# Freebirdgo/MapReduce_Rust

Hardware: AMD Instinct MI355X
Metric: word-count input GB/s (whole node) at 1/2/4/8 MI355X + % of HBM roofline (higher is better)
Workload: dtype u8

## Files before the change

mapreduce_rust_amd/csrc/k_map.hip:

```cpp
#include "mrg_device.h"
#include "mrg_internal.h"
#include "mrg_split.h"

namespace {

constexpr int NW = MRG_MAP_WAVES;
constexpr int WG = 64 * NW;
constexpr int SEG = MRG_MAP_SEG;
constexpr int TILE = MRG_MAP_TILE;
constexpr int HALO = MRG_MAP_HALO;
constexpr int BEHIND = MRG_MAP_BEHIND;
constexpr int NSUB = MRG_MAP_NSUB;
constexpr int BLK = NSUB * TILE;
constexpr int WIN = BEHIND + TILE + HALO + 48;
constexpr int QCAP = TILE / 2 + 16;
constexpr int NMP = 64;
static_assert(TILE == 64 * SEG, "one segment per lane");
static_assert(WIN % 16 == 0, "16-byte window rows");
static_assert(NMP == TILE / SEG, "one mask pair per segment of the tile");
static_assert(16 * (1 + TILE / 16 + HALO / 16) <= WIN, "staged vectors fit the window row");
static_assert(BEHIND + (TILE - 1) + 31 + 20 <= WIN, "the 5-dword key read stays in the window row");
static_assert(BEHIND == 16 && HALO % 16 == 0 && HALO >= 64, "one 16-byte vector behind, whole halo vectors");
static_assert(QCAP >= TILE / 2 + 1, "the token queue holds every start of a tile");
static_assert(BLK == 2 * TILE && NSUB == 2, "A/B register sets hold two tiles per lane (v0, v1)");
// ... 33 lines not shown
    __builtin_amdgcn_wave_barrier();
    __builtin_amdgcn_fence(__ATOMIC_ACQUIRE, "wavefront");
}

#define GAS __attribute__((address_space(1)))
template <class T>
__device__ __forceinline__ GAS T *gp(T *p) {
    return (GAS T *)p;
}
#define CAS __attribute__((address_space(4)))
template <class T>
__device__ __forceinline__ const CAS T *cp(const T *p) {
    return (const CAS T *)p;
}
typedef uint32_t u32x4 __attribute__((ext_vector_type(4)));
typedef uint64_t u64x2 __attribute__((ext_vector_type(2)));
typedef uint32_t u32x3a __attribute__((ext_vector_type(3), aligned(4)));
typedef uint32_t u32x4u __attribute__((ext_vector_type(4), aligned(1)));
typedef uint32_t u32u __attribute__((aligned(1)));
template <class T>
__device__ __forceinline__ T g_add(T *p, T v) {
    return __hip_atomic_fetch_add(gp(p), v, __ATOMIC_RELAXED, __HIP_MEMORY_SCOPE_AGENT);
}
__device__ __forceinline__ uint64_t umin64(uint64_t a, uint64_t b) { return a < b ? a : b; }
__device__ __forceinline__ uint64_t umax64(uint64_t a, uint64_t b) { return a > b ? a : b; }

struct TileInfo {
    uint64_t At, t0, t1, doc_lo, doc_hi, wlo, whi;
    uint32_t docid, v0, v1;
};

struct BlkInfo {
    uint64_t Ab, doc_lo, doc_hi;
    uint32_t docid, v0, v1;
};

__device__ __forceinline__ BlkInfo locate_blk(const MapArgs &A, uint64_t c, uint32_t &d) {
    const CAS uint64_t *cb = cp(A.chunk_base), *doff = cp(A.doc_off);
    while (cb[d + 1] <= c) ++d;
    BlkInfo b;
    b.doc_lo = doff[d];
    b.doc_hi = doff[d + 1];
    b.Ab = (b.doc_lo & ~15ull) + (c - cb[d]) * (uint64_t)BLK;
    b.docid = A.doc_id ? cp(A.doc_id)[d] : d;
    const uint64_t vbase = b.Ab - (uint64_t)BEHIND;
    const uint64_t wlo = umax64(b.doc_lo, b.Ab >= (uint64_t)BEHIND ? b.Ab - BEHIND : 0ull);
    const uint64_t whi = umin64(b.Ab + (uint64_t)(BLK + HALO), b.doc_hi);
    b.v0 = (uint32_t)(((wlo & ~15ull) - vbase) >> 4);
    b.v1 = (uint32_t)((((whi + 15u) & ~15ull) - vbase) >> 4);
    return b;
}

__device__ __forceinline__ uint32_t find_doc(const MapArgs &A, uint64_t c) {
    const CAS uint64_t *cb = cp(A.chunk_base);
    uint32_t lo = 0, hi = A.n_docs;
    while (hi - lo > 1) {
        const uint32_t mid = (lo + hi) >> 1;
        if (cb[mid] <= c) lo = mid;
        else hi = mid;
    }
    return lo;
}

__device__ __forceinline__ TileInfo sub_tile(const BlkInfo &b, uint32_t j) {
    TileInfo t;
    t.At = b.Ab + (uint64_t)j * TILE;
    t.doc_lo = b.doc_lo;
    t.doc_hi = b.doc_hi;
    t.docid = b.docid;
    t.t0 = umax64(t.At, t.doc_lo);
    t.t1 = umin64(t.At + (uint64_t)TILE, t.doc_hi);
    const uint64_t wbase = t.At - (uint64_t)BEHIND;
    t.wlo = umax64(t.doc_lo, t.At >= (uint64_t)BEHIND ? t.At - BEHIND : 0ull);
    t.whi = umin64(t.t1 + (uint64_t)HALO, t.doc_hi);
    t.v0 = (uint32_t)(((t.wlo & ~15ull) - wbase) >> 4);
// ... 442 lines not shown
        for (int t = 0; t < N; ++t) idx[t] = atomicAdd(&(w16[t] ? R.cur16 : R.cur)[b[t]], tl[t] ? 1ull : 0ull);
    } else {
#pragma unroll
        for (int t = 0; t < N; ++t) idx[t] = 0;
    }
    bool anyo = false, ovf[N];
#pragma unroll
    for (int t = 0; t < N; ++t) {
        const bool ok = tl[t] && idx[t] < end[t];
        if (ok) store_tail<IDX>(pool, pool16, w16[t], idx[t], k0[t], k1[t], docid);
        ovf[t] = tl[t] && !ok;
        anyo = anyo || ovf[t];
    }
    if (__any(anyo)) {
#pragma unroll
        for (int t = 0; t < N; ++t)
            if (ovf[t]) ovf_append<IDX>(A, b[t], k0[t], k1[t], docid);
    }
    }
}

template <int CAP, bool IDX, bool WIDE, bool T64>
__device__ __forceinline__ void emit(const MapArgs &A, LdsTable<CAP, IDX> &table, TailRegions R, bool have,
                                     uint64_t tk0, uint64_t tk1, uint32_t tlen, uint64_t tstart, uint32_t traw,
                                     uint32_t docid) {
    const bool is_long = have && tlen > 16u;
    if constexpr (WIDE) {
        wide_store(A, R, have && !is_long, tk0, tk1);
    } else {
    bool tail = false;
    uint32_t h = 0;
    const uint32_t dkey = IDX ? docid : MRG_EMPTY_DOC;
    if (have && !is_long) {
        h = key_hash(tk0, tk1, dkey, A.hash_bits);
    }
    {
        const bool act = have && !is_long && !(map_ablate(A) & 2u);
        tail = (have && !is_long) && !table.insert_wave(act, tk0, tk1, dkey, h);
    }
    if (tail && !(map_ablate(A) & 1u)) {
        const uint32_t b = bucket_of(h);
        const bool w16 = !IDX && (T64 ? (uint32_t)tk1 != 0u : key_over12(tk1));
        if constexpr (!T64) {
            if (w16) {
                tail16_append(A, R, gp(A.pool16), b, tk0, tk1);
            } else {
                const uint64_t ce = atomicAdd(&R.cur[b], 1ull);
                const uint32_t i = (uint32_t)ce;
                if (i < (uint32_t)(ce >> 32)) store_tail32<IDX>(gp(A.pool), i, tk0, tk1, docid);
                else ovf_append<IDX>(A, b, tk0, tk1, docid);
            }
        } else {
        const uint64_t end = (w16 ? R.end16 : R.end)[b];
        const uint64_t idx = atomicAdd(&(w16 ? R.cur16 : R.cur)[b], 1ull);
        if (idx < end) store_tail<IDX>(gp(A.pool), gp(A.pool16), w16, idx, tk0, tk1, docid);
        else ovf_append<IDX>(A, b, tk0, tk1, docid);
        }
    }
    }
    if (__any(is_long)) {
        const uint64_t mask = __ballot(is_long);
        const int leader = __ffsll((long long)mask) - 1;
        uint32_t base = 0;
        if ((int)__lane_id() == leader) base = atomicAdd(R.lcnt, (unsigned int)__popcll(mask));
        base = (uint32_t)__builtin_amdgcn_readlane((int)base, leader);
        const uint32_t k = base + (uint32_t)__popcll(mask & mrg_lanemask_lt());
        if (is_long) {
// ... 83 lines not shown
#define LDS __attribute__((address_space(3)))
__device__ __forceinline__ uint32_t uni_class(const LDS uint8_t *uc, uint32_t cp) {
    uint32_t byte;
    if (cp < 0x800u) byte = uc[cp >> 2];
    else if ((cp >> 8) == 0x20u) byte = uc[512u + ((cp & 255u) >> 2)];
    else return mrg_uclass(cp);
    return (byte >> (2u * (cp & 3u))) & 3u;
}
template <int CAP, bool IDX, bool WIDE, bool T64>
__global__ __launch_bounds__(WG, 1) void k_map(const MapArgs *__restrict__ Ap) {
    const MapArgs &A = *Ap;
    constexpr bool BQ = !IDX && !WIDE;
    constexpr int WROW = BQ ? WINB : WIN, QROW = BQ ? QCAPB : QCAP;
    __shared__ __attribute__((aligned(16))) uint8_t s_win[NW][WROW];
    __shared__ __attribute__((aligned(8))) uint32_t s_mp[NW][BQ ? NMWB : 2 * NMP];
    __shared__ __attribute__((aligned(8))) uint16_t s_q[NW][QROW];
    static_assert((QROW * sizeof(uint16_t)) % 8 == 0 && QROW * sizeof(uint16_t) >= 64 * 8, "queue rows hold 64 u64 slots");
    __shared__ __attribute__((aligned(1024))) uint8_t s_lut[4][256];
    __shared__ __attribute__((aligned(16))) uint32_t s_sel[17 * 17][4];
    __shared__ KeyPair s_key[WIDE ? 2 : CAP];
    __shared__ unsigned int s_cnt[WIDE ? 2 : CAP];
    __shared__ __attribute__((aligned(16))) unsigned int s_doc[IDX ? CAP : 1];
    __shared__ unsigned long long s_tcur[WIDE ? 1 : MRG_NBUCKET];
    __shared__ unsigned long long s_tend[(WIDE || !T64) ? 1 : MRG_NBUCKET];
    __shared__ unsigned long long s_tcur16[(IDX || WIDE) ? 1 : MRG_NBUCKET];
    __shared__ unsigned long long s_tend16[(IDX || WIDE || !T64) ? 1 : MRG_NBUCKET];
    __shared__ uint32_t s_hist[WIDE ? 1 : MRG_NBUCKET + 1];
    __shared__ unsigned int s_wcur[WIDE ? MRG_WMAP_MAXB1 : 1];
    __shared__ __attribute__((aligned(16))) uint64_t s_wspl[WIDE ? 2 * MRG_WMAP_MAXB1 : 1];
    __shared__ __attribute__((aligned(4))) uint8_t s_wix[WIDE ? MRG_WMAP_IXR * MRG_WIDE_IX1 : 4];
    __shared__ uint32_t s_next, s_ngen;
    __shared__ uint32_t s_stolen;
    __shared__ uint32_t s_share[2];
    __shared__ uint32_t s_pool[NW];
    __shared__ uint32_t s_nuni;
    __shared__ uint8_t s_uc[9 * 64];
    __shared__ uint32_t s_tot[3];
    __shared__ unsigned int s_fill;
    __shared__ unsigned int s_lcnt;
    __shared__ unsigned int s_door[(MRG_MAP_DOOR && !WIDE) ? LdsTable<CAP, IDX>::DW : 1];
    static_assert(WIDE || sizeof(s_q) >= CAP * sizeof(uint16_t), "flush ranks reuse the queues");
    static_assert((CAP & (CAP - 1)) == 0 && CAP >= 64 && CAP <= 65536, "2-way sets: NS = CAP / 2 a power of two, ranks in u16");
    static_assert(sizeof(s_door) / sizeof(s_door[0]) >= ((MRG_MAP_DOOR && !WIDE) ? LdsTable<CAP, IDX>::DW : 1u), "doorkeeper words");
    static_assert(!WIDE || (sizeof(s_wcur) / sizeof(s_wcur[0]) == MRG_WMAP_MAXB1 && sizeof(s_wspl) / sizeof(s_wspl[0]) == 2 * MRG_WMAP_MAXB1 &&
                            sizeof(s_wix) == MRG_WMAP_IXR * MRG_WIDE_IX1 && MRG_WIDE_IX1 % 4 == 0),
                  "wide map: cursors, splitters and index rows as the host plan sizes them");
    if constexpr (WIDE) {
        if (A.wR * A.wB1r > (uint32_t)MRG_WMAP_MAXB1 || A.wB1r == 0u || (A.wix && A.wR > (uint32_t)MRG_WMAP_IXR)) return;
    }

    const int tid = threadIdx.x;
    const int lane = tid & 63, wv = __builtin_amdgcn_readfirstlane(tid >> 6);
    if constexpr (WIDE) {
        const uint32_t nb1 = A.wR * A.wB1r, nsp = 2u * A.wR * (A.wB1r - 1u);
        for (uint32_t b = tid; b < nb1; b += WG) s_wcur[b] = 0;
        for (uint32_t i = tid; i < nsp; i += WG) s_wspl[i] = gp(A.wspl)[i];
        if (A.wix)
            for (uint32_t i = tid; i < A.wR * (MRG_WIDE_IX1 / 4); i += WG)
                reinterpret_cast<uint32_t *>(s_wix)[i] = gp(reinterpret_cast<const uint32_t *>(A.wix))[i];
    }
    for (int i = tid; i < (WIDE ? 2 : CAP); i += WG) {
        s_key[i] = KeyPair{MRG_EMPTY_K0, MRG_EMPTY_K1};
        s_cnt[i] = 0;
        if (IDX) s_doc[i] = MRG_EMPTY_DOC;
    }
    if (MRG_MAP_DOOR && !WIDE)
// ... 29 lines not shown
        s_tot[1] = 0;
        s_tot[2] = 0;
        s_fill = 0;
        s_lcnt = 0;
    }
    for (int i = tid; i < 9 * 64; i += WG) {
        const uint32_t blk = i < 512 ? (uint32_t)i >> 6 : 0x20u;
        s_uc[i] = c_uclass_stage2[c_uclass_stage1[blk] * 64u + ((uint32_t)i & 63u)];
    }
    for (int i = tid; i < 1024; i += WG) {
        const uint32_t v = (uint32_t)i & 255u, c = mrg_uclass(v & 127u);
        const uint32_t ws = v >= 128u ? 0x11u : ((c == MRG_CLS_W ? 1u : 0u) | (c == MRG_CLS_S ? 0x10u : 0u));
        s_lut[i >> 8][v] = (uint8_t)(ws << (i >> 8));
    }
    auto zmask = [](uint32_t L, uint32_t j) {
        uint32_t m = 0;
        for (uint32_t p = 0; p < 4; ++p)
            if (4u * j + 3u - p >= L) m |= 0xFFu << (8u * p);
        return m;
    };
    for (int i = tid; i < 17 * 17 * 4; i += WG) {
        const uint32_t L = (uint32_t)i / 68u, g = ((uint32_t)i / 4u) % 17u, j = (uint32_t)i & 3u;
        const uint32_t zm = zmask(L, j), gm = zmask(g, j);
        s_sel[L * 17u + g][j] = ((0x00010203u + (gm & 0x01010101u)) & ~zm) | (0x0C0C0C0Cu & zm);
    }
    LdsTable<CAP, IDX> table{s_key, s_cnt, s_doc, s_door, &s_fill};
    const TailRegions tails{s_tcur, s_tend, s_tcur16, s_tend16, &s_lcnt, s_wcur, s_wspl, A.wix ? s_wix : nullptr};
    uint32_t my_tokens = 0;
#ifdef MRG_MAP_ABLATION
    const uint32_t abl = A.ablate;
#else
    constexpr uint32_t abl = MRG_MAP_ABL_CONST;
#endif
    const uint32_t hbits = A.hash_bits;
    GAS uint64_t *const pool = gp(A.pool);
    GAS uint64_t *const pool16 = gp(A.pool16);
    uint8_t *win = s_win[wv];
    uint32_t *mw = s_mp[wv];
    uint64_t *mp = reinterpret_cast<uint64_t *>(s_mp[wv]);
    uint16_t *queue = s_q[wv];
    __syncthreads();

    const uint32_t j0 = 1u + (uint32_t)lane;
    const uint32_t j1 = lane == 0 ? 0u : 64u + (uint32_t)lane;
    const bool has1 = lane < 5;
    auto load = [&](const TileInfo &t, uint4 &p0, uint4 &p1) {
        const GAS u32x4 *src = reinterpret_cast<const GAS u32x4 *>(gp(A.in) + (t.At - (uint64_t)BEHIND));
        u32x4 v0 = {0, 0, 0, 0}, v1 = {0, 0, 0, 0};
        if (j0 >= t.v0 && j0 < t.v1) v0 = src[j0];
        if (has1 && j1 >= t.v0 && j1 < t.v1) v1 = src[j1];
        p0 = uint4{v0.x, v0.y, v0.z, v0.w};
        p1 = uint4{v1.x, v1.y, v1.z, v1.w};
    };
    struct Blk {
        uint4 v0, v1, e;
    };
#ifdef MRG_MAP_ABLATION
    BlkInfo first_blk{};
#endif
    auto load_blk = [&](const BlkInfo &b0, Blk &X) {
#ifdef MRG_MAP_ABLATION
        const BlkInfo &b = (abl & 8u) ? first_blk : b0;
#else
        const BlkInfo &b = b0;
#endif
        const GAS uint8_t *src = gp(A.in) + (b.Ab - (uint64_t)BEHIND);
        auto ld = [&](uint32_t idx) -> uint4 {
            const u32x4 t = __builtin_nontemporal_load(reinterpret_cast<const GAS u32x4 *>(src + 16u * min(max(idx, b.v0), b.v1 - 1u)));
            return uint4{t.x, t.y, t.z, t.w};
        };
        X.v0 = ld(1u + (uint32_t)lane);
        X.v1 = ld(65u + (uint32_t)lane);
        X.e = ld(lane == 0 ? 0u : 128u + (uint32_t)lane);
    };

    GAS uint32_t *glist = gp(A.gbits) + (uint64_t)blockIdx.x * A.kwords;

#ifdef MRG_MAP_PROF
    const bool P = A.prof != nullptr;
    uint64_t pacc[7] = {0, 0, 0, 0, 0, 0, 0}, tl = P ? clock64() : 0;
    const uint64_t wg_t0 = wall_clock64();
    unsigned long long ftv[5] = {0, 0, 0, 0, 0};
#define MRG_FT(i)                                   \
    if (P && tid == 0) ftv[i] = wall_clock64();
#define MRG_PT(i)                          \
    if (P) {                               \
        const uint64_t t_ = clock64();     \
        pacc[i] += t_ - tl;                \
        tl = t_;                           \
    }
#else
#define MRG_PT(i)
#define MRG_FT(i)
#endif
    auto extract = [&](uint32_t q, uint32_t sraw, uint32_t total, bool &fast, bool &slow, uint32_t &s,
                       uint64_t &tk0, uint64_t &tk1) -> uint32_t {
        const bool act = q < total;
        s = act ? sraw : 0u;
        uint32_t Wp, Sp;
        if constexpr (BQ) {
            const uint32_t ma = mw[s >> 4], mb = mw[(s >> 4) + 1u];
            Wp = __builtin_amdgcn_perm(mb, ma, 0x05040100u);
            Sp = __builtin_amdgcn_perm(mb, ma, 0x07060302u);
        } else {
            const uint64_t pr = mp[s >> 4];
            Wp = (uint32_t)pr;
            Sp = (uint32_t)(pr >> 32);
        }
        const uint32_t i = s & 15u;
// ... 71 lines not shown
                const uint32_t r = (uint32_t)__builtin_ctz(~(W >> b));
                W &= ~(((1u << r) - 1u) << b);
                const uint32_t off = (uint32_t)BEHIND + 16u * seg + b;
                const uint32_t dw = off >> 2, ra = off & 3u;
                const uint32_t d0 = win32[dw], d1 = win32[dw + 1], d2 = win32[dw + 2], d3 = win32[dw + 3],
                               d4 = win32[dw + 4];
                const u32x4 sl = *reinterpret_cast<const u32x4 *>(s_sel[r * 17u + 16u]);
                const uint32_t a0 = __builtin_amdgcn_alignbyte(d1, d0, ra), a1 = __builtin_amdgcn_alignbyte(d2, d1, ra),
                               a2 = __builtin_amdgcn_alignbyte(d3, d2, ra), a3 = __builtin_amdgcn_alignbyte(d4, d3, ra),
                               a4 = __builtin_amdgcn_alignbyte(0u, d4, ra);
                const uint64_t v0 = ((uint64_t)__builtin_amdgcn_perm(a1, a0, sl.x) << 32) | __builtin_amdgcn_perm(a2, a1, sl.y);
                const uint64_t v1 = ((uint64_t)__builtin_amdgcn_perm(a3, a2, sl.z) << 32) | __builtin_amdgcn_perm(a4, a3, sl.w);
                const uint32_t ks = 8u * tlen;
                if (ks == 0u) {
                    tk0 |= v0;
                    tk1 |= v1;
                } else if (ks < 64u) {
                    tk0 |= v0 >> ks;
                    tk1 |= (v1 >> ks) | (v0 << (64u - ks));
                } else {
                    tk1 |= v0 >> (ks - 64u);
                }
                tlen += r;
            }
            tlen += (uint32_t)__builtin_popcount(W);
            if (S) {
                traw = 16u * seg + e - s;
                return true;
            }
        }
        return false;
    };

    auto process_blk = [&](const BlkInfo &I, const Blk &X, uint32_t cblk, auto &&mid) {
        const uint64_t Ab = I.Ab, doc_lo = I.doc_lo, doc_hi = I.doc_hi;
        const uint32_t docid = I.docid;
        const uint32_t lo_rel = doc_lo > Ab ? (uint32_t)(doc_lo - Ab) : 0u;
        const uint32_t hi_rel = (uint32_t)umin64(doc_hi - Ab, (uint64_t)(BLK + HALO));
        const bool edge = lo_rel != 0u || hi_rel != (uint32_t)(BLK + HALO);
        auto clip = [&](uint32_t m, uint32_t B) -> uint32_t {
            const uint32_t lo_inv = lo_rel > B ? min(lo_rel - B, 16u) : 0u;
            const uint32_t hi_ok = B < hi_rel ? min(hi_rel - B, 16u) : 0u;
            const uint32_t valid = ((1u << hi_ok) - 1u) & ~((1u << lo_inv) - 1u);
            return (m & (valid | (valid << 16))) | ((~valid & 0xFFFFu) << 16);
        };
        auto classify = [&](const uint4 &x) -> uint32_t {
            uint32_t e[16];
#pragma unroll
            for (int k = 0; k < 4; ++k) {
                const uint32_t w = k == 0 ? x.x : (k == 1 ? x.y : (k == 2 ? x.z : x.w));
#pragma unroll
                for (int b = 0; b < 4; ++b)
                    e[4 * k + b] = s_lut[b][b == 0 ? (w & 0xFFu) : (b == 3 ? w >> 24 : __builtin_amdgcn_ubfe(w, 8 * b, 8))];
            }
            uint32_t yk[4];
#pragma unroll
            for (int k = 0; k < 4; ++k) yk[k] = e[4 * k] | e[4 * k + 1] | e[4 * k + 2] | e[4 * k + 3];
            const uint32_t y = (yk[0] | (yk[1] << 8)) | ((yk[2] | (yk[3] << 8)) << 16);
            const uint32_t t = y & 0x0F0F0F0Fu, u = (y >> 4) & 0x0F0F0F0Fu;
            return __builtin_amdgcn_perm(u | (u >> 4), t | (t >> 4), 0x06040200u);
        };
        auto na = [](const uint4 &x) { return ((x.x | x.y | x.z | x.w) & 0x80808080u) != 0u; };
        const uint32_t l16 = (uint32_t)lane * SEG;
        uint32_t m0 = classify(X.v0), m1 = classify(X.v1);
        uint32_t mh;
        {
            const uint32_t e0 = lane_u32(X.e.x, 1), e1 = lane_u32(X.e.y, 1), e2 = lane_u32(X.e.z, 1),
                           e3 = lane_u32(X.e.w, 1);
            const uint32_t k = (uint32_t)lane & 15u;
            const uint32_t dwv = k < 8u ? (k < 4u ? e0 : e1) : (k < 12u ? e2 : e3);
            const uint32_t cl = s_lut[0][__builtin_amdgcn_ubfe(dwv, 8u * (k & 3u), 8)];
            const uint32_t wm = (uint32_t)__ballot(lane < 16 && (cl & 1u));
            const uint32_t sm = (uint32_t)__ballot(lane < 16 && (cl & 0x10u));
            mh = (wm & 0xFFFFu) | (sm << 16);
        }
        if (edge) {
            m0 = clip(m0, l16);
            m1 = clip(m1, 1024u + l16);
            mh = clip(mh, (uint32_t)BLK);
        }
        const bool n0 = na(X.v0), n1 = na(X.v1), ne = na(X.e);
        uint32_t prev_blk =
            Ab > doc_lo ? (uint32_t)(s_lut[0][lane_u32(X.e.w, 0) >> 24] >> 4) & 1u : 1u;
        bool defer_blk = false;
        if (!(abl & 256u) && !(MRG_MAP_ABL_CONST & 0x20000u) && __any(n0 || n1 || (lane <= 1 && ne))) {
#ifdef MRG_MAP_NO_UNI
            defer_blk = true;
#else
            const int64_t dlo = (int64_t)(doc_lo - Ab);
            const int lo = (int)(dlo < -(int64_t)BEHIND ? -(int64_t)BEHIND : dlo);
            const int hi = (int)umin64(doc_hi - Ab, (uint64_t)(BLK + HALO));
            const LDS uint8_t *uc = (const LDS uint8_t *)s_uc;
            bool bad = false;
            auto hb = [](uint32_t d) { return ((((d & 0x80808080u) >> 7) * 0x00204081u) >> 21) & 0xFu; };
            auto nam_of = [](uint32_t m) { return m & (m >> 16) & 0xFFFFu; };
            auto leads = [&](const uint4 &x, uint32_t nam) {
                return (hb(x.x & (x.x << 1)) | (hb(x.y & (x.y << 1)) << 4) | (hb(x.z & (x.z << 1)) << 8) |
                        (hb(x.w & (x.w << 1)) << 12)) & nam;
            };
            const uint32_t nam0 = nam_of(m0), nam1 = nam_of(m1), namh_w = nam_of(mh);
            const uint32_t ld0 = leads(X.v0, nam0), ld1 = leads(X.v1, nam1);
            uint4 xh{0u, 0u, 0u, 0u};
            uint32_t namh = 0u, ldh = 0u;
            if (namh_w) {
                xh = uint4{lane_u32(X.e.x, 1), lane_u32(X.e.y, 1), lane_u32(X.e.z, 1), lane_u32(X.e.w, 1)};
                if (lane == 63) {
                    namh = namh_w;
                    ldh = leads(xh, namh);
                }
            }
            const uint32_t before = lane_u32(X.e.w, 0);
            int pbp = 0;
            bool has_b = false;
            if (dlo < 0 && (before >> 24) >= 0x80u) {
                uint32_t bb = before >> 24;
                pbp = -1;
                for (int k = 2; k <= 4 && (bb & 0xC0u) == 0x80u; ++k) {
                    bb = (before >> (8 * (4 - k))) & 0xFFu;
                    pbp = -k;
                }
                if (bb < 0xC0u || pbp < lo) bad = true;
                else has_b = true;
            }
            const uint32_t v1_first = lane_u32(X.v1.x, 0), halo_next = lane_u32(X.e.x, 2);
            uint32_t nA = from_next_lane(X.v0.x), nB = from_next_lane(X.v1.x);
            if (lane == 63) {
                nA = v1_first;
                nB = xh.x;
            }
            auto dec = [&](uint32_t p, uint32_t d0, uint32_t d1, uint32_t d2, uint32_t d3, uint32_t d4, int so,
                           uint32_t &W, uint32_t &S, uint32_t &C) {
                const uint32_t k = p >> 2;
                const uint32_t a = (k & 2u) ? ((k & 1u) ? d3 : d2) : ((k & 1u) ? d1 : d0);
                const uint32_t b = (k & 2u) ? ((k & 1u) ? d4 : d3) : ((k & 1u) ? d2 : d1);
                const uint32_t w = __builtin_amdgcn_alignbyte(b, a, p & 3u);
                auto rd = [&](uint64_t x) -> uint32_t { return (w >> (8u * (uint32_t)x)) & 0xFFu; };
                uint32_t cp = 0, raw;
                const int n = mrg_utf8_decode(rd, 0ull, (uint64_t)min(hi - (so + (int)p), 4), &cp, &raw);
                bad |= n == 0;
                const uint32_t span = ((1u << n) - 1u) << p;
                const uint32_t cl = uni_class(uc, cp);
                C |= span;
                W |= cl == MRG_CLS_W ? span : 0u;
                S |= cl == MRG_CLS_S ? span : 0u;
            };
            uint32_t W0 = 0, S0 = 0, C0 = 0, W1 = 0, S1 = 0, C1 = 0;
            uint32_t mAB0 = (MRG_MAP_ABL_CONST & 0x10000u) ? 0u : (ld0 | (ld1 << 16));
// ... 94 lines not shown
                Wh = WE;
                Sh = SE;
                Ch = CE;
            }
            const uint32_t sp0 = pack(W0, S0, C0), sp1 = pack(W1, S1, C1);
            uint32_t in0 = from_prev_lane(sp0), in1 = from_prev_lane(sp1);
            const uint32_t sp0_last = lane_u32(sp0, 63);
            if (lane == 0) {
                in0 = bsp;
                in1 = sp0_last;
            }
            auto fix = [&](uint32_t m, uint32_t nam, uint32_t W, uint32_t S, uint32_t C, uint32_t in) -> uint32_t {
                W = (W | ((in >> 4) & 0xFu)) & 0xFFFFu;
                S = (S | ((in >> 8) & 0xFu)) & 0xFFFFu;
                C = (C | (in & 0xFu)) & 0xFFFFu;
                if (!(MRG_MAP_ABL_CONST & 0x10000u)) bad |= C != nam;
                return ((m & 0xFFFFu & ~nam) | W) | ((((m >> 16) & ~nam) | S) << 16);
            };
            m0 = fix(m0, nam0, W0, S0, C0, in0);
            m1 = fix(m1, nam1, W1, S1, C1, in1);
            uint32_t mh_l = mh;
            if (lane == 63) mh_l = fix(mh, namh, Wh, Sh, Ch, sp1);
            mh = lane_u32(mh_l, 63);
            prev_blk = lane_u32(pb_l, 0);
            defer_blk = __any(bad);
            if (!defer_blk && lane == 0) atomicAdd(&s_nuni, Ab + (uint64_t)TILE < doc_hi ? 2u : 1u);
#endif
        }
        MRG_PT(1);
        mid();
        MRG_PT(0);
        if (defer_blk) {
            if (lane == 0) {
                for (uint32_t j = 0; j < NSUB && Ab + (uint64_t)j * TILE < doc_hi; ++j) {
                    const uint32_t k = atomicAdd(&s_ngen, 1u);
                    if (k < A.kwords) glist[k] = (uint32_t)(cblk * NSUB + j);
                }
            }
            return;
        }
        if (abl & 32u) {
            my_tokens += (m0 ^ m1 ^ mh ^ prev_blk) & 1u;
            return;
        }

        auto rounds = [&](uint32_t total, bool may_claim) -> uint32_t {
            uint32_t nslow = 0;
            for (uint32_t base = 0; base < total; base += 128) {
                bool fa, sa, fb, sb;
                uint32_t sA, sB;
                uint64_t a0, a1, b0, b1;
                const uint32_t qa = base + (uint32_t)lane, qb = qa + 64u;
                const uint32_t ra = queue[min(qa, (uint32_t)QROW - 1u)], rb = queue[min(qb, (uint32_t)QROW - 1u)];
                uint32_t ga = extract(qa, ra, total, fa, sa, sA, a0, a1);
                uint32_t gb = extract(qb, rb, total, fb, sb, sB, b0, b1);
                if (!(abl & 1024u) && __any((ga | gb) != 0u)) {
                    squeeze(ga, a0, a1);
                    squeeze(gb, b0, b1);
                }
                const uint64_t ma = __ballot(sa), mb = __ballot(sb);
                if (ma | mb) {
                    const uint32_t ra = __builtin_amdgcn_mbcnt_hi((uint32_t)(ma >> 32), __builtin_amdgcn_mbcnt_lo((uint32_t)ma, 0u));
                    const uint32_t rb = __builtin_amdgcn_mbcnt_hi((uint32_t)(mb >> 32), __builtin_amdgcn_mbcnt_lo((uint32_t)mb, 0u));
                    const uint32_t na = (uint32_t)__builtin_popcountll(ma);
                    if (sa) queue[nslow + ra] = (uint16_t)sA;
                    if (sb) queue[nslow + na + rb] = (uint16_t)sB;
// ... 17 lines not shown
            wave_sync_lds();
            auto rd = [&](uint64_t a) -> uint32_t {
                if (a >= At && a < whi) return (uint32_t)win[a - wbase];
                return (uint32_t)gp(A.in)[a];
            };
            for (uint32_t base = 0; base < nslow; base += 64) {
                const uint32_t q = base + (uint32_t)lane;
                bool have = false;
                uint64_t tk0 = 0, tk1 = 0, a = 0;
                uint32_t tlen = 0, traw = 0;
                if (q < nslow) {
                    const uint32_t s = queue[q];
                    a = At + s;
                    if (!(abl & 128u) && mask_walk(s, nseg, tk0, tk1, tlen, traw)) {
                        have = tlen > 0;
                    } else {
                        uint64_t e2;
                        if (walk_token(rd, a, doc_hi, A.counters, tk0, tk1, tlen, e2) && tlen > 0) {
                            have = true;
                            traw = (uint32_t)(e2 - a);
                        }
                    }
                }
                my_tokens += have ? 1u : 0u;
                emit<CAP, IDX, WIDE, T64>(A, table, tails, have, tk0, tk1, tlen, a, traw, docid);
            }
        };
        auto table_open = [&]() -> bool {
            return __builtin_amdgcn_readfirstlane(__hip_atomic_load(&s_fill, __ATOMIC_RELAXED, __HIP_MEMORY_SCOPE_WORKGROUP)) <
                   (uint32_t)CAP;
        };

        if constexpr (BQ) {
            const uint64_t whi = umin64(Ab + (uint64_t)(BLK + HALO), doc_hi);
            wave_sync_lds();
            reinterpret_cast<uint4 *>(win)[1 + lane] = X.v0;
            reinterpret_cast<uint4 *>(win)[65 + lane] = X.v1;
            if (lane >= 1 && lane < 5) reinterpret_cast<uint4 *>(win)[128 + lane] = X.e;
            mw[lane] = m0;
            mw[64 + lane] = m1;
            if (lane == 0) mw[2 * 64] = mh;
            uint32_t pv0 = from_prev_lane(m0) >> 31, pv1 = from_prev_lane(m1) >> 31;
            const uint32_t m0_last = lane_u32(m0, 63) >> 31;
            if (lane == 0) {
                pv0 = prev_blk;
                pv1 = m0_last;
            }
            const uint32_t S0 = m0 >> 16, S1 = m1 >> 16;
            uint32_t st0 = ~S0 & ((S0 << 1) | pv0) & 0xFFFFu;
            uint32_t st1 = ~S1 & ((S1 << 1) | pv1) & 0xFFFFu;
            if (abl & 64u) {
                my_tokens += (st0 ^ st1) & 1u;
                st0 = 0;
                st1 = 0;
            }
            my_tokens += (abl & 4u) ? (uint32_t)__builtin_popcount(st0 | (st1 << 16)) : 0u;
            uint32_t pos0, pos1;
            auto scan2 = [&](uint32_t a0, uint32_t a1) -> uint32_t {
                const uint32_t c0 = (uint32_t)__builtin_popcount(a0), c1 = (uint32_t)__builtin_popcount(a1);
                const uint32_t incl = wave_incl_scan(c0 | (c1 << 16));
                const uint32_t tot = lane_u32(incl, 63);
                pos0 = (incl & 0xFFFFu) - c0;
                pos1 = (tot & 0xFFFFu) + (incl >> 16) - c1;
                return (abl & 68u) ? 0u : (tot & 0xFFFFu) + (tot >> 16);
            };
            auto in_range = [&](uint32_t lo, uint32_t hi, uint32_t &a0, uint32_t &a1) {
                const uint32_t g0 = (uint32_t)lane, g1 = 64u + (uint32_t)lane;
                a0 = g0 >= lo && g0 < hi ? st0 : 0u;
                a1 = g1 >= lo && g1 < hi ? st1 : 0u;
            };
            uint32_t a0 = st0, a1 = st1, seg_hi = BLK / SEG;
            uint32_t total = scan2(a0, a1);
            if (total > (uint32_t)QCAPB) {
                seg_hi = QRANGE;
                in_range(0u, seg_hi, a0, a1);
                total = scan2(a0, a1);
            }
// ... 84 lines not shown
        const uint64_t c0 = (uint64_t)first_u32(s_share[0]) + (uint64_t)first_u32(r);
        if (c0 < (uint64_t)whi_b) {
            run_cur = (uint32_t)c0 + 1u;
            run_end = (uint32_t)umin64(c0 + R, (uint64_t)whi_b);
            return (uint32_t)c0;
        }
        const uint64_t ns2 = A.n_static, np = A.n_chunks - ns2;
        wave_sync_lds();
        uint32_t pt = first_u32(s_pool[wv]);
        while ((pt >> 8) < 8u) {
            const uint32_t part = pt & 7u;
            uint32_t k = 0;
            if (lane == 0) k = atomicAdd(&s_stolen, (uint32_t)MRG_MAP_STEAL_K);
            if (first_u32(k) + (uint32_t)MRG_MAP_STEAL_K > A.steal_max) {
                pt = 8u << 8;
                break;
            }
            const uint32_t plo = (uint32_t)(np * part / 8u), phi = (uint32_t)(np * (part + 1u) / 8u);
            unsigned long long q = 0;
            if (lane == 0) q = atomicAdd(&A.pool_ctr[16u * part], (unsigned long long)MRG_MAP_STEAL_K);
            const uint32_t at = plo + first_u32((uint32_t)umin64(q, 0xFFFFFFFFull));
            if (at < phi) {
                if (lane == 0) s_pool[wv] = pt;
                run_cur = (uint32_t)ns2 + at + 1u;
                run_end = (uint32_t)ns2 + min(phi, at + (uint32_t)MRG_MAP_STEAL_K);
                if (cp(A.chunk_base)[dcur] > ns2 + at) dcur = find_doc(A, ns2 + at);
                return (uint32_t)ns2 + at;
            }
            pt = ((pt & 7u) + 1u) % 8u | (((pt >> 8) + 1u) << 8);
        }
        if (lane == 0) s_pool[wv] = pt;
        return NONE;
    };
    auto next_blk = [&](const BlkInfo &P, uint32_t cp_, uint32_t cn) -> BlkInfo {
        if (cn != cp_ + 1u || P.Ab + (uint64_t)BLK >= P.doc_hi) return locate_blk(A, cn, dcur);
        BlkInfo b = P;
        b.Ab = P.Ab + (uint64_t)BLK;
        const uint64_t whi = umin64(b.Ab + (uint64_t)(BLK + HALO), b.doc_hi);
        b.v0 = 0u;
        b.v1 = (uint32_t)((((whi + 15u) & ~15ull) - (b.Ab - (uint64_t)BEHIND)) >> 4);
        return b;
    };
    uint32_t c = grab();
    if (c != NONE) dcur = find_doc(A, c);
    Blk XA, XB;
    BlkInfo IA{}, IB{};
    auto settle = [](Blk &X) {
        asm volatile("" : "+v"(X.v0.x), "+v"(X.v0.y), "+v"(X.v0.z), "+v"(X.v0.w), "+v"(X.v1.x), "+v"(X.v1.y),
                     "+v"(X.v1.z), "+v"(X.v1.w), "+v"(X.e.x), "+v"(X.e.y), "+v"(X.e.z), "+v"(X.e.w));
    };
    if (c != NONE) {
        IA = locate_blk(A, c, dcur);
#ifdef MRG_MAP_ABLATION
        first_blk = IA;
#endif
        load_blk(IA, XA);
        settle(XA);
    }
    while (c != NONE) {
        const uint32_t cB = grab();
        IB = cB != NONE ? next_blk(IA, c, cB) : IA;
        load_blk(IB, XB);
        process_blk(IA, XA, c, [&]() { settle(XB); });
        c = cB;
        if (c == NONE) break;
        const uint32_t cA = grab();
        IA = cA != NONE ? next_blk(IB, c, cA) : IB;
        load_blk(IA, XA);
        process_blk(IB, XB, c, [&]() { settle(XA); });
        c = cA;
    }
    MRG_PT(4);
#ifdef MRG_MAP_PROF
    __shared__ unsigned long long s_loop_end;
    if (tid == 0) s_loop_end = 0;
    lds_only_barrier();
    if (P && lane == 0) atomicMax(&s_loop_end, (unsigned long long)wall_clock64());
#endif
    lds_only_barrier();
    if (s_ngen) __syncthreads();
    {
        const uint32_t ng = min(s_ngen, A.kwords);
        for (uint32_t i = (uint32_t)wv; i < ng; i += NW) {
            {
                const uint32_t kk = first_u32(glist[i]);
                const uint64_t cb = kk / NSUB;
                uint32_t dgen = find_doc(A, cb);
                const BlkInfo b = locate_blk(A, cb, dgen);
                const TileInfo T = sub_tile(b, kk % NSUB);
                uint4 x0, x1;
                load(T, x0, x1);
                wave_sync_lds();
                if (j0 >= T.v0 && j0 < T.v1) reinterpret_cast<uint4 *>(win)[j0] = x0;
                if (has1 && j1 >= T.v0 && j1 < T.v1) reinterpret_cast<uint4 *>(win)[j1] = x1;
                wave_sync_lds();
                my_tokens += generic_tile<CAP, IDX, WIDE, T64>(A, table, tails, win, T.At, T.t0, T.t1,
                                                    T.doc_lo, T.doc_hi, T.wlo, T.whi, T.docid);
            }
        }
    }

    MRG_PT(5);
    lds_only_barrier();
    uint32_t my_tail = 0, my_tail16 = 0;
    if constexpr (WIDE) {
        uint32_t over = 0;
        for (uint32_t b = tid; b < A.wR * A.wB1r; b += WG) {
            const uint32_t n = s_wcur[b];
            gp(A.wcnt)[(uint64_t)b * gridDim.x + blockIdx.x] = n;
            my_tail += n;
            over += n > A.wcap ? n - A.wcap : 0u;
        }
        if (over) g_add(&A.counters[CNT_OVF], (unsigned long long)over);
    } else {
    uint16_t *s_rank = &s_q[0][0];
    GAS uint32_t *bcount = gp(A.bcount) + (uint64_t)blockIdx.x * MRG_NBUCKET;
    for (int b = tid; b < MRG_NBUCKET; b += WG) {
        const uint32_t n = T64 ? (uint32_t)(s_tcur[b] - (s_tend[b] - gp(A.bcap)[b]))
                               : (uint32_t)s_tcur[b] - ((uint32_t)(s_tcur[b] >> 32) - gp(A.bcap)[b]);
        my_tail += n;
        bcount[b] = n;
        if (!IDX) {
            const uint32_t n16 = T64 ? (uint32_t)(s_tcur16[b] - (s_tend16[b] - gp(A.bcap16)[b]))
                                     : (uint32_t)s_tcur16[b] - ((uint32_t)(s_tcur16[b] >> 32) - gp(A.bcap16)[b]);
            my_tail += n16;
            my_tail16 += n16;
            gp(A.bcount16)[(uint64_t)blockIdx.x * MRG_NBUCKET + b] = n16;
        }
    }
    for (int b = tid; b <= MRG_NBUCKET; b += WG) s_hist[b] = 0;
    lds_only_barrier();
    MRG_FT(0);
    for (int i = tid; i < CAP; i += WG) {
        const KeyPair k = s_key[i];
        if (k.a == MRG_EMPTY_K0) continue;
        const uint32_t b = bucket_of(key_hash(k.a, k.b, IDX ? s_doc[i] : MRG_EMPTY_DOC, A.hash_bits));
        s_rank[i] = (uint16_t)atomicAdd(&s_hist[b], 1u);
    }
    lds_only_barrier();
    MRG_FT(1);
    if (tid < 64) {
        uint32_t run = 0;
        for (int b0 = 0; b0 < MRG_NBUCKET; b0 += 64) {
            const uint32_t v = s_hist[b0 + lane];
            const uint32_t inc = wave_incl_scan(v);
            s_hist[b0 + lane] = run + inc - v;
            run += lane_u32(inc, 63);
        }
        if (lane == 0) s_hist[MRG_NBUCKET] = run;
    }
    lds_only_barrier();
    MRG_FT(2);
    GAS uint32_t *foff = gp(A.foff) + (uint64_t)blockIdx.x * (MRG_NBUCKET + 1);
    for (int b = tid; b <= MRG_NBUCKET; b += WG) foff[b] = s_hist[b];
    const uint64_t reg = (uint64_t)blockIdx.x * CAP;
    for (int i = tid; i < CAP; i += WG) {
        const KeyPair k = s_key[i];
        if (k.a == MRG_EMPTY_K0) continue;
        const uint32_t d = IDX ? s_doc[i] : MRG_EMPTY_DOC;
        const uint32_t b = bucket_of(key_hash(k.a, k.b, d, A.hash_bits));
        const uint64_t pos2 = reg + s_hist[b] + s_rank[i];
        gp(A.fk0)[pos2] = k.a;
        gp(A.fk1)[pos2] = k.b;
        gp(A.fcnt)[pos2] = s_cnt[i];
        if (IDX) gp(A.fdoc)[pos2] = d;
    }
    }
    MRG_FT(3);
    uint32_t t = my_tokens, ttl = my_tail, t16 = my_tail16;
    for (int off = 32; off > 0; off >>= 1) {
        t += __shfl_down(t, off);
        ttl += __shfl_down(ttl, off);
        t16 += __shfl_down(t16, off);
    }
    if (lane == 0) {
        atomicAdd(&s_tot[0], t);
        atomicAdd(&s_tot[1], ttl);
        if (t16) atomicAdd(&s_tot[2], t16);
    }
    lds_only_barrier();
    if (tid == 0) {
        g_add(&A.counters[CNT_TOKENS], (unsigned long long)s_tot[0]);
        g_add(&A.counters[CNT_REC], (unsigned long long)s_tot[1]);
        if (s_tot[2]) g_add(&A.counters[CNT_REC16], (unsigned long long)s_tot[2]);
        if (s_ngen + s_nuni) g_add(&A.counters[CNT_NONASCII], (unsigned long long)(s_ngen + s_nuni));
        if (s_ngen > A.kwords) g_add(&A.counters[CNT_OVF], (unsigned long long)(s_ngen - A.kwords));
        gp(A.lcount)[blockIdx.x] = s_lcnt;
        if (s_lcnt) g_add(&A.counters[CNT_LONG], (unsigned long long)s_lcnt);
    }
    MRG_FT(4);
    MRG_PT(6);
#ifdef MRG_MAP_PROF
    if (P && lane == 0) {
// ... 165 lines not shown
```

mapreduce_rust_amd/csrc/mrgpu.cpp:

```cpp
#include <sys/stat.h>

#include <rccl/rccl.h>

#include <fcntl.h>
#include <unistd.h>

#include <atomic>
#include <condition_variable>
#include <exception>
#include <memory>
#include <thread>

#include "mrg_host.h"

using namespace mrg_host;

static_assert(sizeof(XRec) == MRG_XREC_BYTES, "exchange record layout (include/mrgpu.h)");

thread_local std::string mrg_host::g_err;

DeviceCache &DeviceCache::get() {
    static DeviceCache *c = new DeviceCache();
    return *c;
}
// ... 1121 lines not shown
        uint64_t *d_rbase16 = att.get<uint64_t>(MRG_NBUCKET);
        uint32_t *d_bcap16 = att.get<uint32_t>(MRG_NBUCKET);
        A.bcount16 = att.get<uint32_t>((uint64_t)grid * MRG_NBUCKET);
        MapArgs *dargs = att.get<MapArgs>(1);
        if (ocap > 0xFFFFFFF0ull) raise(MRG_ENOMEM, "input too large for one map launch");
        A.ovf = att.get<uint64_t>((uint64_t)MRG_NBUCKET * ocap * RW);
        A.onext = att.get<uint32_t>(MRG_NBUCKET);
        A.ocap = (uint32_t)ocap;
        stage_fill(c, A.onext, 0, 4ull * MRG_NBUCKET);
        stage_h2d(c, d_rbase, rbase.data(), 8ull * MRG_NBUCKET);
        stage_h2d(c, d_bcap, bcap32.data(), 4ull * MRG_NBUCKET);
        stage_h2d(c, d_rbase16, rbase16.data(), 8ull * MRG_NBUCKET);
        stage_h2d(c, d_bcap16, bcap16_32.data(), 4ull * MRG_NBUCKET);
        A.rbase = d_rbase; A.bcap = d_bcap; A.rbase16 = d_rbase16; A.bcap16 = d_bcap16;
        A.pool = att.get<uint64_t>((rtot * MRG_TAIL_BYTES(idx) + 16 + 7) / 8);
        A.pool16 = att.get<uint64_t>(2 * rtot16 + 2);
        A.fk0 = att.get<uint64_t>((uint64_t)grid * cap);
        A.fk1 = att.get<uint64_t>((uint64_t)grid * cap);
        A.fcnt = att.get<uint32_t>((uint64_t)grid * cap);
        A.fdoc = idx ? att.get<uint32_t>((uint64_t)grid * cap) : nullptr;
        A.foff = att.get<uint32_t>((uint64_t)grid * (MRG_NBUCKET + 1));
        const uint64_t lslots = map_args_shared(c, att, A, in, ms, lcap, launches == 0, launches);
        A.ablate = getenv("MRG_ABLATE") ? (uint32_t)atoi(getenv("MRG_ABLATE")) : 0u;
        A.prof = nullptr;
        if (getenv("MRG_PROF")) {
            A.prof = att.get<unsigned long long>(8 + 8ull * grid);
            HIPCHK(hipMemsetAsync(A.prof, 0, 8ull * (8 + 8ull * grid), s));
        }
        stage_fill(c, c->d_cnt, 0, sizeof(unsigned long long) * CNT_N);
        stage_fill(c, &c->d_cnt[CNT_ERRPOS], 0xFF, sizeof(unsigned long long));
        stage_h2d(c, dargs, &A, sizeof(MapArgs));
        flush_stage(c);
        ev_rec(c, c->ev, 0);
        const bool tail64 = !map_tail_packed(rtot, rtot16, ms) || env_u64("MRG_TEST_TAIL64", 0) != 0;
        mrg_launch_map(nullptr, dargs, c->app, grid, c->lds_cap, s, false, tail64);
        ev_rec(c, c->ev, 1);
        HIPCHK(hipGetLastError());
        ++launches;
        if (launches == 1 && !idx && (c->spec_agg || cold_repeats) && !A.prof && !wide_forced() &&
            !getenv("MRG_NO_SPEC_AGG") && grid <= 2048) {
            ev_rec(c, c->ev, 2);
            uint32_t nsub = c->agg_nsub;
            if (const uint64_t t = env_u64("MRG_TEST_AGG_NSUB", 0)) nsub = (uint32_t)t;
            const bool c32 = c->spec_agg ? c->spec_c32 : true;
            spec = agg_launch(c, A, (uint32_t)grid, cap, agg_ocap(c), nsub, lslots, c32 && grid <= 512, false);
        }
        uint32_t *onext = (uint32_t *)&c->h_cnt[CNT_N + 8];
        HIPCHK(hipMemcpyAsync(onext, A.onext, 4ull * MRG_NBUCKET, hipMemcpyDeviceToHost, s));
        read_counters(c);
        c->st.map_spill = 0;
        for (int b = 0; b < MRG_NBUCKET; ++b) c->st.map_spill += std::min<uint64_t>(onext[b], ocap);
        if (A.prof) {
            unsigned long long pr[8];
            HIPCHK(hipMemcpy(pr, A.prof, sizeof pr, hipMemcpyDeviceToHost));
            double tot = 0;
            for (int i = 0; i < 7; ++i) tot += (double)pr[i];
            static const char *nm[7] = {"load-wait", "classify", "stage+scan+queue", "token rounds", "slow tokens",
                                        "non-ascii", "flush"};
            fprintf(stderr, "[mrgpu] map phase clocks (sum over waves %.3e):", tot);
            for (int i = 0; i < 7; ++i) fprintf(stderr, " %s %.1f%%", nm[i], 100.0 * (double)pr[i] / (tot > 0 ? tot : 1));
            fprintf(stderr, "\n");
            std::vector<unsigned long long> wt(8ull * grid);
            HIPCHK(hipMemcpy(wt.data(), A.prof + 8, 8ull * wt.size(), hipMemcpyDeviceToHost));
            if (wt[1]) {
                unsigned long long t0 = ~0ull, t1 = 0, ls = 0;
                std::vector<double> dur(grid), end(grid), lend(grid);
                std::vector<std::vector<double>> fst(5, std::vector<double>(grid, 0.0));
// ... 2058 lines not shown
```

Before: 1468.

## Slim per-block state in map loop and specialize hash bits on tail mode

Replaces the two full BlkInfo register sets in the double-buffered map loop with one compact CurBlk. When the next chunk is not the consecutive one, its metadata is passed through a small per-wave LDS slot and read back as scalars. It also makes hash_bits a compile-time zero for the packed-tail variant (the host forces the 64-bit tail path whenever hash_bits is nonzero), and uses opaque lane values to simplify lane predicates. The aim is lower VGPR/SGPR pressure and fewer 64-bit ops in the hot loop, at the cost of an extra LDS round-trip and wave sync on non-consecutive chunk switches.

```diff
diff --git a/mapreduce_rust_amd/csrc/k_map.hip b/mapreduce_rust_amd/csrc/k_map.hip
--- a/mapreduce_rust_amd/csrc/k_map.hip
+++ b/mapreduce_rust_amd/csrc/k_map.hip
@@ -89,8 +89,23 @@
 
 struct BlkInfo {
     uint64_t Ab, doc_lo, doc_hi;
-    uint32_t docid, v0, v1;
+    uint32_t docid, v0, v1, cend;
 };
+
+struct CurBlk {
+    uint64_t Ab, doc_hi;
+    int32_t lo;
+    uint32_t docid;
+    uint32_t cend;
+};
+__device__ __forceinline__ CurBlk cur_of(const BlkInfo &b) {
+    const int64_t d = (int64_t)(b.doc_lo - b.Ab);
+    return CurBlk{b.Ab, b.doc_hi, (int32_t)(d < -(int64_t)BEHIND ? -(int64_t)BEHIND : d), b.docid, b.cend};
+}
+__device__ __forceinline__ uint32_t clip_u32(uint64_t x, uint32_t m) {
+    const uint32_t l = (uint32_t)(x >> 32) ? 0xFFFFFFFFu : (uint32_t)x;
+    return l < m ? l : m;
+}
 
 __device__ __forceinline__ BlkInfo locate_blk(const MapArgs &A, uint64_t c, uint32_t &d) {
     const CAS uint64_t *cb = cp(A.chunk_base), *doff = cp(A.doc_off);
@@ -98,6 +113,7 @@
     BlkInfo b;
     b.doc_lo = doff[d];
     b.doc_hi = doff[d + 1];
+    b.cend = (uint32_t)cb[d + 1];
     b.Ab = (b.doc_lo & ~15ull) + (c - cb[d]) * (uint64_t)BLK;
     b.docid = A.doc_id ? cp(A.doc_id)[d] : d;
     const uint64_t vbase = b.Ab - (uint64_t)BEHIND;
@@ -606,7 +622,7 @@
     uint32_t h = 0;
     const uint32_t dkey = IDX ? docid : MRG_EMPTY_DOC;
     if (have && !is_long) {
-        h = key_hash(tk0, tk1, dkey, A.hash_bits);
+        h = key_hash(tk0, tk1, dkey, T64 ? A.hash_bits : 0u);
     }
     {
         const bool act = have && !is_long && !(map_ablate(A) & 2u);
@@ -756,6 +772,7 @@
     __shared__ uint32_t s_next, s_ngen;
     __shared__ uint32_t s_stolen;
     __shared__ uint32_t s_share[2];
+    __shared__ __attribute__((aligned(16))) uint32_t s_nxt[NW][8];
     __shared__ uint32_t s_pool[NW];
     __shared__ uint32_t s_nuni;
     __shared__ uint8_t s_uc[9 * 64];
@@ -851,7 +868,7 @@
 #else
     constexpr uint32_t abl = MRG_MAP_ABL_CONST;
 #endif
-    const uint32_t hbits = A.hash_bits;
+    const uint32_t hbits = T64 ? A.hash_bits : 0u;
     GAS uint64_t *const pool = gp(A.pool);
     GAS uint64_t *const pool16 = gp(A.pool16);
     uint8_t *win = s_win[wv];
@@ -874,14 +891,18 @@
     struct Blk {
         uint4 v0, v1, e;
     };
+    struct BlkLoad {
+        uint64_t Ab;
+        uint32_t v0, v1;
+    };
 #ifdef MRG_MAP_ABLATION
-    BlkInfo first_blk{};
-#endif
-    auto load_blk = [&](const BlkInfo &b0, Blk &X) {
+    BlkLoad first_blk{};
+#endif
+    auto load_blk = [&](const BlkLoad &b0, Blk &X) {
 #ifdef MRG_MAP_ABLATION
-        const BlkInfo &b = (abl & 8u) ? first_blk : b0;
+        const BlkLoad &b = (abl & 8u) ? first_blk : b0;
 #else
-        const BlkInfo &b = b0;
+        const BlkLoad &b = b0;
 #endif
         const GAS uint8_t *src = gp(A.in) + (b.Ab - (uint64_t)BEHIND);
         auto ld = [&](uint32_t idx) -> uint4 {
@@ -893,7 +914,7 @@
         X.e = ld(lane == 0 ? 0u : 128u + (uint32_t)lane);
     };
 
-    GAS uint32_t *glist = gp(A.gbits) + (uint64_t)blockIdx.x * A.kwords;
+    auto glist_of = [&]() -> GAS uint32_t * { return gp(A.gbits) + (uint64_t)blockIdx.x * A.kwords; };
 
 #ifdef MRG_MAP_PROF
     const bool P = A.prof != nullptr;
@@ -1031,11 +1052,12 @@
         return false;
     };
 
-    auto process_blk = [&](const BlkInfo &I, const Blk &X, uint32_t cblk, auto &&mid) {
-        const uint64_t Ab = I.Ab, doc_lo = I.doc_lo, doc_hi = I.doc_hi;
+    auto process_blk = [&](const CurBlk &I, const Blk &X, uint32_t cblk, auto &&mid) {
+        const uint64_t Ab = I.Ab, doc_hi = I.doc_hi;
         const uint32_t docid = I.docid;
-        const uint32_t lo_rel = doc_lo > Ab ? (uint32_t)(doc_lo - Ab) : 0u;
-        const uint32_t hi_rel = (uint32_t)umin64(doc_hi - Ab, (uint64_t)(BLK + HALO));
+        const int lo = I.lo;
+        const uint32_t lo_rel = lo > 0 ? (uint32_t)lo : 0u;
+        const uint32_t hi_rel = clip_u32(doc_hi - Ab, (uint32_t)(BLK + HALO));
         const bool edge = lo_rel != 0u || hi_rel != (uint32_t)(BLK + HALO);
         auto clip = [&](uint32_t m, uint32_t B) -> uint32_t {
             const uint32_t lo_inv = lo_rel > B ? min(lo_rel - B, 16u) : 0u;
@@ -1061,16 +1083,18 @@
         };
         auto na = [](const uint4 &x) { return ((x.x | x.y | x.z | x.w) & 0x80808080u) != 0u; };
         const uint32_t l16 = (uint32_t)lane * SEG;
+        uint32_t ln = (uint32_t)lane;
+        asm volatile("" : "+v"(ln));
         uint32_t m0 = classify(X.v0), m1 = classify(X.v1);
         uint32_t mh;
         {
             const uint32_t e0 = lane_u32(X.e.x, 1), e1 = lane_u32(X.e.y, 1), e2 = lane_u32(X.e.z, 1),
                            e3 = lane_u32(X.e.w, 1);
-            const uint32_t k = (uint32_t)lane & 15u;
+            const uint32_t k = ln & 15u;
             const uint32_t dwv = k < 8u ? (k < 4u ? e0 : e1) : (k < 12u ? e2 : e3);
             const uint32_t cl = s_lut[0][__builtin_amdgcn_ubfe(dwv, 8u * (k & 3u), 8)];
-            const uint32_t wm = (uint32_t)__ballot(lane < 16 && (cl & 1u));
-            const uint32_t sm = (uint32_t)__ballot(lane < 16 && (cl & 0x10u));
+            const uint32_t wm = (uint32_t)__ballot((cl & 1u) != 0u);
+            const uint32_t sm = (uint32_t)__ballot((cl & 0x10u) != 0u);
             mh = (wm & 0xFFFFu) | (sm << 16);
         }
         if (edge) {
@@ -1080,15 +1104,13 @@
         }
         const bool n0 = na(X.v0), n1 = na(X.v1), ne = na(X.e);
         uint32_t prev_blk =
-            Ab > doc_lo ? (uint32_t)(s_lut[0][lane_u32(X.e.w, 0) >> 24] >> 4) & 1u : 1u;
+            lo < 0 ? (uint32_t)(s_lut[0][lane_u32(X.e.w, 0) >> 24] >> 4) & 1u : 1u;
         bool defer_blk = false;
-        if (!(abl & 256u) && !(MRG_MAP_ABL_CONST & 0x20000u) && __any(n0 || n1 || (lane <= 1 && ne))) {
+        if (!(abl & 256u) && !(MRG_MAP_ABL_CONST & 0x20000u) && __any(n0 || n1 || (ln <= 1u && ne))) {
 #ifdef MRG_MAP_NO_UNI
             defer_blk = true;
 #else
-            const int64_t dlo = (int64_t)(doc_lo - Ab);
-            const int lo = (int)(dlo < -(int64_t)BEHIND ? -(int64_t)BEHIND : dlo);
-            const int hi = (int)umin64(doc_hi - Ab, (uint64_t)(BLK + HALO));
+            const int hi = (int)hi_rel;
             const LDS uint8_t *uc = (const LDS uint8_t *)s_uc;
             bool bad = false;
             auto hb = [](uint32_t d) { return ((((d & 0x80808080u) >> 7) * 0x00204081u) >> 21) & 0xFu; };
@@ -1111,7 +1133,7 @@
             const uint32_t before = lane_u32(X.e.w, 0);
             int pbp = 0;
             bool has_b = false;
-            if (dlo < 0 && (before >> 24) >= 0x80u) {
+            if (lo < 0 && (before >> 24) >= 0x80u) {
                 uint32_t bb = before >> 24;
                 pbp = -1;
                 for (int k = 2; k <= 4 && (bb & 0xC0u) == 0x80u; ++k) {
@@ -1272,6 +1294,7 @@
         MRG_PT(0);
         if (defer_blk) {
             if (lane == 0) {
+                GAS uint32_t *glist = glist_of();
                 for (uint32_t j = 0; j < NSUB && Ab + (uint64_t)j * TILE < doc_hi; ++j) {
                     const uint32_t k = atomicAdd(&s_ngen, 1u);
                     if (k < A.kwords) glist[k] = (uint32_t)(cblk * NSUB + j);
@@ -1355,17 +1378,17 @@
         };
 
         if constexpr (BQ) {
-            const uint64_t whi = umin64(Ab + (uint64_t)(BLK + HALO), doc_hi);
+            const uint64_t whi = Ab + (uint64_t)clip_u32(doc_hi - Ab, (uint32_t)(BLK + HALO));
             wave_sync_lds();
             reinterpret_cast<uint4 *>(win)[1 + lane] = X.v0;
             reinterpret_cast<uint4 *>(win)[65 + lane] = X.v1;
-            if (lane >= 1 && lane < 5) reinterpret_cast<uint4 *>(win)[128 + lane] = X.e;
+            if (ln - 1u < 4u) reinterpret_cast<uint4 *>(win)[128 + lane] = X.e;
             mw[lane] = m0;
             mw[64 + lane] = m1;
-            if (lane == 0) mw[2 * 64] = mh;
+            if (ln == 0u) mw[2 * 64] = mh;
             uint32_t pv0 = from_prev_lane(m0) >> 31, pv1 = from_prev_lane(m1) >> 31;
             const uint32_t m0_last = lane_u32(m0, 63) >> 31;
-            if (lane == 0) {
+            if (ln == 0u) {
                 pv0 = prev_blk;
                 pv1 = m0_last;
             }
@@ -1516,43 +1539,66 @@
         if (lane == 0) s_pool[wv] = pt;
         return NONE;
     };
-    auto next_blk = [&](const BlkInfo &P, uint32_t cp_, uint32_t cn) -> BlkInfo {
-        if (cn != cp_ + 1u || P.Ab + (uint64_t)BLK >= P.doc_hi) return locate_blk(A, cn, dcur);
-        BlkInfo b = P;
-        b.Ab = P.Ab + (uint64_t)BLK;
-        const uint64_t whi = umin64(b.Ab + (uint64_t)(BLK + HALO), b.doc_hi);
-        b.v0 = 0u;
-        b.v1 = (uint32_t)((((whi + 15u) & ~15ull) - (b.Ab - (uint64_t)BEHIND)) >> 4);
-        return b;
-    };
     uint32_t c = grab();
     if (c != NONE) dcur = find_doc(A, c);
     Blk XA, XB;
-    BlkInfo IA{}, IB{};
+    CurBlk I{};
+    uint32_t *nxt = s_nxt[wv];
     auto settle = [](Blk &X) {
         asm volatile("" : "+v"(X.v0.x), "+v"(X.v0.y), "+v"(X.v0.z), "+v"(X.v0.w), "+v"(X.v1.x), "+v"(X.v1.y),
                      "+v"(X.v1.z), "+v"(X.v1.w), "+v"(X.e.x), "+v"(X.e.y), "+v"(X.e.z), "+v"(X.e.w));
     };
+    auto want_of = [&]() { return c + 1u < I.cend ? c + 1u : c; };
+    auto step = [&](const Blk &Xc, Blk &Xn) {
+        uint32_t cn = grab();
+        const uint32_t want = want_of();
+        BlkLoad L;
+        if (cn == want) {
+            const uint32_t hi = clip_u32(I.doc_hi - (I.Ab + (uint64_t)BLK), (uint32_t)(BLK + HALO));
+            L = BlkLoad{I.Ab + (uint64_t)BLK, 0u, ((hi + 15u) >> 4) + 1u};
+        } else if (cn != NONE) {
+            const BlkInfo b = locate_blk(A, cn, dcur);
+            L = BlkLoad{b.Ab, b.v0, b.v1};
+            const CurBlk n = cur_of(b);
+            if (lane == 0) {
+                *reinterpret_cast<uint4 *>(nxt) = uint4{(uint32_t)n.Ab, (uint32_t)(n.Ab >> 32), (uint32_t)n.doc_hi,
+                                                        (uint32_t)(n.doc_hi >> 32)};
+                *reinterpret_cast<uint4 *>(nxt + 4) = uint4{(uint32_t)n.lo, n.docid, n.cend, 0u};
+            }
+        } else {
+            L = BlkLoad{I.Ab, 1u, 2u};
+        }
+        load_blk(L, Xn);
+        process_blk(I, Xc, c, [&]() { settle(Xn); });
+        asm volatile("" : "+s"(cn));
+        if (cn == want_of()) {
+            I.Ab += (uint64_t)BLK;
+            I.lo = -(int32_t)BEHIND;
+        } else if (cn != NONE) {
+            wave_sync_lds();
+            const uint4 r0 = *reinterpret_cast<const uint4 *>(nxt), r1 = *reinterpret_cast<const uint4 *>(nxt + 4);
+            I.Ab = (uint64_t)first_u32(r0.x) | ((uint64_t)first_u32(r0.y) << 32);
+            I.doc_hi = (uint64_t)first_u32(r0.z) | ((uint64_t)first_u32(r0.w) << 32);
+            I.lo = (int32_t)first_u32(r1.x);
+            I.docid = first_u32(r1.y);
+            I.cend = first_u32(r1.z);
+        }
+        c = cn;
+    };
     if (c != NONE) {
-        IA = locate_blk(A, c, dcur);
+        const BlkInfo b = locate_blk(A, c, dcur);
+        I = cur_of(b);
+        const BlkLoad L{b.Ab, b.v0, b.v1};
 #ifdef MRG_MAP_ABLATION
-        first_blk = IA;
-#endif
-        load_blk(IA, XA);
+        first_blk = L;
+#endif
+        load_blk(L, XA);
         settle(XA);
     }
     while (c != NONE) {
-        const uint32_t cB = grab();
-        IB = cB != NONE ? next_blk(IA, c, cB) : IA;
-        load_blk(IB, XB);
-        process_blk(IA, XA, c, [&]() { settle(XB); });
-        c = cB;
+        step(XA, XB);
         if (c == NONE) break;
-        const uint32_t cA = grab();
-        IA = cA != NONE ? next_blk(IB, c, cA) : IB;
-        load_blk(IA, XA);
-        process_blk(IB, XB, c, [&]() { settle(XA); });
-        c = cA;
+        step(XB, XA);
     }
     MRG_PT(4);
 #ifdef MRG_MAP_PROF
@@ -1565,6 +1611,7 @@
     if (s_ngen) __syncthreads();
     {
         const uint32_t ng = min(s_ngen, A.kwords);
+        const GAS uint32_t *glist = glist_of();
         for (uint32_t i = (uint32_t)wv; i < ng; i += NW) {
             {
                 const uint32_t kk = first_u32(glist[i]);
@@ -1618,7 +1665,7 @@
     for (int i = tid; i < CAP; i += WG) {
         const KeyPair k = s_key[i];
         if (k.a == MRG_EMPTY_K0) continue;
-        const uint32_t b = bucket_of(key_hash(k.a, k.b, IDX ? s_doc[i] : MRG_EMPTY_DOC, A.hash_bits));
+        const uint32_t b = bucket_of(key_hash(k.a, k.b, IDX ? s_doc[i] : MRG_EMPTY_DOC, hbits));
         s_rank[i] = (uint16_t)atomicAdd(&s_hist[b], 1u);
     }
     lds_only_barrier();
@@ -1642,7 +1689,7 @@
         const KeyPair k = s_key[i];
         if (k.a == MRG_EMPTY_K0) continue;
         const uint32_t d = IDX ? s_doc[i] : MRG_EMPTY_DOC;
-        const uint32_t b = bucket_of(key_hash(k.a, k.b, d, A.hash_bits));
+        const uint32_t b = bucket_of(key_hash(k.a, k.b, d, hbits));
         const uint64_t pos2 = reg + s_hist[b] + s_rank[i];
         gp(A.fk0)[pos2] = k.a;
         gp(A.fk1)[pos2] = k.b;
diff --git a/mapreduce_rust_amd/csrc/mrgpu.cpp b/mapreduce_rust_amd/csrc/mrgpu.cpp
--- a/mapreduce_rust_amd/csrc/mrgpu.cpp
+++ b/mapreduce_rust_amd/csrc/mrgpu.cpp
@@ -1177,7 +1177,7 @@
         stage_h2d(c, dargs, &A, sizeof(MapArgs));
         flush_stage(c);
         ev_rec(c, c->ev, 0);
-        const bool tail64 = !map_tail_packed(rtot, rtot16, ms) || env_u64("MRG_TEST_TAIL64", 0) != 0;
+        const bool tail64 = !map_tail_packed(rtot, rtot16, ms) || A.hash_bits != 0 || env_u64("MRG_TEST_TAIL64", 0) != 0;
         mrg_launch_map(nullptr, dargs, c->app, grid, c->lds_cap, s, false, tail64);
         ev_rec(c, c->ev, 1);
         HIPCHK(hipGetLastError());
```

Result: faster. 1508, median of 6 (+2.7%).
